# Wang-Xiaoyang/resource_packing_self_play

Hardware: AMD Instinct MI355X
Metric: self-play episodes/sec (with MCTS node expansions/sec alongside) (higher is better)
Workload: dtype f64 PUCT / f32 Q + CNN, u32 bit-board

## Files before the change

resource_packing_self_play_amd/csrc/rp_engine.hip:

```cpp
#include <hip/hip_runtime.h>
#include <math.h>
#include <stdarg.h>
#include <stdint.h>
#include <stdio.h>
#include <stdlib.h>
#include <string.h>

#include <algorithm>
#include <string>
#include <utility>
#include <vector>

#include "../../include/rp_engine.h"

#pragma clang fp contract(off)

typedef unsigned long long u64;
typedef unsigned int u32;
typedef unsigned short u16;
typedef unsigned char u8;

#define NONE32 0xFFFFFFFFu
#define NSA_MASK 0x3FFFFFFFu
#define WAVES_PER_BLOCK 4
// ... 2615 lines not shown
                if constexpr (e == 0 || T::L.s[e > 0 ? e - 1 : 0] != s) {
                    constexpr int s2 = s + 2;
                    const int off = s2 < 18 ? fbase + s2 * 2048 : fnext + (s2 - 18) * 2048;
                    wq[s2 % 3][0] = rs_load_b(frs, voff, off); wq[s2 % 3][1] = rs_load_b(frs, voff, off + 1024);
                }
                if constexpr (e + 2 < NE) bq[(e + 2) % 3] = b_read(std::integral_constant<int, (e + 2 < NE ? e + 2 : 0)>{});
                const f32x4 w0 = wq[s % 3][0], w1 = wq[s % 3][1], b = bq[e % 3];
                __builtin_amdgcn_sched_barrier(0);
#pragma unroll
                for (int j = 0; j < 4; ++j) {
                    acc[k][0] = __builtin_amdgcn_mfma_f32_16x16x4f32(w0[j], b[j], acc[k][0], 0, 0, 0);
                    acc[k][1] = __builtin_amdgcn_mfma_f32_16x16x4f32(w1[j], b[j], acc[k][1], 0, 0, 0);
                }
                __builtin_amdgcn_sched_barrier(0);
            });
            pm_sync<S>();
            const f32x4 ba = *(const f32x4 *)(sbias + 32 * kc + 4 * g), bb = *(const f32x4 *)(sbias + 32 * kc + 16 + 4 * g);
            if (kc < 3) {
                if (kc == 1)
                    pm_for<NP>([&](auto K) {
                        constexpr int k = decltype(K)::value, p = T::L.pos[k];
                        xs[k][0] = (acc[k][0] + ba) + xs[k][0]; xs[k][1] = (acc[k][1] + bb) + xs[k][1];
                        *(f32x4 *)(wb0 + p * 512) = rs_relu(xs[k][0]); *(f32x4 *)(wb1 + p * 512) = rs_relu(xs[k][1]);
                        __builtin_amdgcn_sched_barrier(0);
                    });
                else
                    pm_for<NP>([&](auto K) {
                        constexpr int k = decltype(K)::value, p = T::L.pos[k];
                        *(f32x4 *)(wb0 + p * 512) = rs_relu(acc[k][0] + ba); *(f32x4 *)(wb1 + p * 512) = rs_relu(acc[k][1] + bb);
                        __builtin_amdgcn_sched_barrier(0);
                    });
                pm_sync<S>();
            } else {
                const __amdgpu_buffer_rsrc_t ors = __builtin_amdgcn_make_buffer_rsrc((void *)(out + (size_t)leaf0 * PIX * 32), 0, nbytes, RS_BUF_FLAGS);
                pm_for<NP>([&](auto K) {
                    constexpr int k = decltype(K)::value, p = T::L.pos[k];
                    acc[k][0] = (acc[k][0] + ba) + xs[k][0]; acc[k][1] = (acc[k][1] + bb) + xs[k][1];
                    __builtin_amdgcn_raw_buffer_store_b128(__builtin_bit_cast(u32x4, acc[k][0]), ors, xoff, p * 128, RS_STREAM_AUX);
                    __builtin_amdgcn_raw_buffer_store_b128(__builtin_bit_cast(u32x4, acc[k][1]), ors, xoff, p * 128 + 64, RS_STREAM_AUX);
                    __builtin_amdgcn_sched_barrier(0);
                });
                if (out_relu != nullptr) {
                    const __amdgpu_buffer_rsrc_t rrs = __builtin_amdgcn_make_buffer_rsrc((void *)(out_relu + (size_t)leaf0 * PIX * 32), 0, nbytes, RS_BUF_FLAGS);
                    pm_for<NP>([&](auto K) {
                        constexpr int k = decltype(K)::value, p = T::L.pos[k];
                        __builtin_amdgcn_raw_buffer_store_b128(__builtin_bit_cast(u32x4, rs_relu(acc[k][0])), rrs, xoff, p * 128, RS_STREAM_AUX);
                        __builtin_amdgcn_raw_buffer_store_b128(__builtin_bit_cast(u32x4, rs_relu(acc[k][1])), rrs, xoff, p * 128 + 64, RS_STREAM_AUX);
                        __builtin_amdgcn_sched_barrier(0);
                    });
                }
            }
        }
    }
}
template <int S>
__global__ void __launch_bounds__(256, 2) k_resstage32_pm(const float *__restrict__ x, const float *__restrict__ frag, const float *__restrict__ bias,
                                                          float *__restrict__ out, float *__restrict__ out_relu, long long B, const int *__restrict__ nrows_dev) {
    extern __shared__ __attribute__((aligned(16))) float rb_lds[];
    const int wv = wave_in_block();
    if (nrows_dev) { const long long n = *nrows_dev; if (n < B) B = n; }
    float *sbias = rb_lds;
    if constexpr (S == 3) {
        if ((long long)blockIdx.x * 64 >= B) return;
        for (int i = threadIdx.x; i < 128; i += blockDim.x) sbias[i] = bias[i];
        __syncthreads();
        const long long leaf0 = ((long long)blockIdx.x * 4 + wv) * 16;
        if (leaf0 >= B) return;
        pm_body<3, 0>(x, frag, out, out_relu, B, leaf0, (long long)gridDim.x * 64, sbias, rb_lds + 128 + (size_t)wv * PM_IMG_FLOATS(3));
    } else {
        if ((long long)blockIdx.x * 16 >= B) return;
        for (int i = threadIdx.x; i < 128; i += blockDim.x) sbias[i] = bias[i];
        __syncthreads();
        const long long leaf0 = (long long)blockIdx.x * 16, stride = (long long)gridDim.x * 16;
        float *img = rb_lds + 128;
        switch (wv) {
            case 0: pm_body<5, 0>(x, frag, out, out_relu, B, leaf0, stride, sbias, img); break;
            case 1: pm_body<5, 1>(x, frag, out, out_relu, B, leaf0, stride, sbias, img); break;
            case 2: pm_body<5, 2>(x, frag, out, out_relu, B, leaf0, stride, sbias, img); break;
            default: pm_body<5, 3>(x, frag, out, out_relu, B, leaf0, stride, sbias, img); break;
        }
    }
}

#define CP_PS 36
#ifdef CP_STAMP
__device__ unsigned long long g_cp_stamp[8];
#endif
template <int NT, int CIN, bool TAIL = false>
__global__ void __launch_bounds__(256, 2) k_convpool32(const float *__restrict__ x, const float *__restrict__ frag, const float *__restrict__ bias,
                                                       float *__restrict__ out, long long B, int S_h, int S_w, int IMGW, int wave_floats,
                                                       const int *__restrict__ nrows_dev) {
    constexpr int XQ = CIN / 16;
    constexpr int PS = CP_PS;
    extern __shared__ __attribute__((aligned(16))) float rb_lds[];
    const int lane = lane_id(), wv = wave_in_block();
    if (nrows_dev) { const long long n = *nrows_dev; if (n < B) B = n; }
    if (((long long)blockIdx.x * 4) * IMGW >= B) return;
    const int PW = r32_pw(S_w), PIX = S_h * S_w, IMGP = r32_imgp(S_h, S_w), MP = IMGW * PIX;
    const int Hp = (S_h + 1) >> 1, Wp = (S_w + 1) >> 1, PP = Hp * Wp;
    constexpr int NTT = NT + (TAIL ? 1 : 0);
    int *ptab = (int *)rb_lds;
    int *pool = ptab + 16 * NTT;
    float *img = rb_lds + 16 * NTT + ((IMGW * PP + 3) & ~3) + (size_t)wv * wave_floats;
    for (int i = threadIdx.x; i < 16 * NTT; i += blockDim.x) {
        int im = i / PIX, pq = i - im * PIX, r = pq / S_w, c = pq - r * S_w;
        ptab[i] = i < MP ? im * IMGP + (r + 1) * PW + c + 1 : 0;
    }
    for (int i = threadIdx.x; i < IMGW * PP; i += blockDim.x) {
        int im = i / PP, pp = i - im * PP, pr = pp / Wp, px = pp - pr * Wp;
        pool[i] = (im * IMGP + (2 * pr + 1) * PW + 2 * px + 1) | ((pr > 0) << 16) | ((2 * pr + 1 < S_h) << 17) | ((px > 0) << 18) | ((2 * px + 1 < S_w) << 19);
    }
    {
        float4 *z4 = (float4 *)img;
        for (int i = lane; i < wave_floats / 4; i += 64) z4[i] = make_float4(0.f, 0.f, 0.f, 0.f);
    }
    __syncthreads();
    const long long stride_leaves = (long long)gridDim.x * 4 * IMGW;
    long long leaf0 = ((long long)blockIdx.x * 4 + wv) * IMGW;
    if (leaf0 >= B) return;
    const int n = lane & 15, g = lane >> 4;
    int abase[NT], pin[NT];
#pragma unroll
    for (int t = 0; t < NT; ++t) {
        const int m = t * 16 + n, pc = m < MP ? ptab[m] : IMGW * IMGP;
        abase[t] = (ptab[m < MP ? m : 0] - (PW + 1)) * PS + CIN / 4 * g;
        pin[t] = pc * PS + 4 * g;
    }
    const __amdgpu_buffer_rsrc_t frs = __builtin_amdgcn_make_buffer_rsrc((void *)frag, 0, 9 * CIN * 32 * 4, RS_BUF_FLAGS);
    const f32x4 ba = *(const f32x4 *)(bias + 4 * g), bb = *(const f32x4 *)(bias + 16 + 4 * g);
    const int rowoff = n * (CIN * 4) + g * 16;
    auto task_bytes = [&](long long l0) { return (int)(B - l0 < IMGW ? B - l0 : IMGW) * PIX * CIN * 4; };
    f32x4 xv[NT][XQ], wq[3][2];
    int t_abase = 0, t_voff0 = 0, t_voff1 = 0;
    f32x4 t_acc = (f32x4){0.f, 0.f, 0.f, 0.f}, t_w0[2], t_w1[2];
    const int cg = lane >> 3, kk = (lane >> 2) & 1, mt = 16 * NT + (lane & 3);
    int pout_t = 0, pin_t = 0;
    f32x4 xvt = (f32x4){0.f, 0.f, 0.f, 0.f};
    const int xq_t = (lane >> 2) & (CIN / 4 - 1);
    const int rowoff_t = (lane & 3) * (CIN * 4) + xq_t * 16;
    if (TAIL) {
        const int pc = mt < MP ? ptab[mt] : IMGW * IMGP;
        t_abase = (ptab[mt < MP ? mt : 0] - (PW + 1)) * PS + (CIN / 2) * kk;
        const int lw = 4 * (cg & 3) + (lane & 3) + 32 * kk;
        t_voff0 = (cg >> 2) * 1024 + lw * 16; t_voff1 = (cg >> 2) * 1024 + (lw + 16) * 16;
        pout_t = pc * PS + 4 * cg;
        pin_t = pc * PS + 4 * xq_t;
    }
    auto load_x = [&](long long l0) {
        const __amdgpu_buffer_rsrc_t rs = __builtin_amdgcn_make_buffer_rsrc((void *)(x + (size_t)l0 * PIX * CIN), 0, task_bytes(l0), RS_BUF_FLAGS);
#pragma unroll
        for (int t = 0; t < NT; ++t)
#pragma unroll
            for (int q = 0; q < XQ; ++q) xv[t][q] = rs_load_x(rs, rowoff, t * 16 * CIN * 4 + 64 * q);
        if (TAIL) xvt = rs_load_x(rs, rowoff_t, NT * 16 * CIN * 4);
    };
    const int cq = lane & 7;
    load_x(leaf0);
    wq[0][0] = rs_load_b(frs, lane * 16, 0); wq[0][1] = rs_load_b(frs, lane * 16, 1024);
    wq[1][0] = rs_load_b(frs, lane * 16, 2048); wq[1][1] = rs_load_b(frs, lane * 16, 3072);
    if (TAIL) {
        t_w0[0] = rs_load_b(frs, t_voff0, 0); t_w1[0] = rs_load_b(frs, t_voff1, 0);
        t_w0[1] = rs_load_b(frs, t_voff0, 2048); t_w1[1] = rs_load_b(frs, t_voff1, 2048);
    }
#ifdef CP_STAMP
    unsigned long long st_acc[8] = {0, 0, 0, 0, 0, 0, 0, 0}, st_last = __builtin_amdgcn_s_memtime();
#define CP_T(k) { unsigned long long now_ = __builtin_amdgcn_s_memtime(); st_acc[k] += now_ - st_last; st_last = now_; }
// ... 325 lines not shown
    u64 *meta_id;
    double *meta_bl;
    u8 *meta_has;
    int64_t meta_cap;
    int n_cu = 256;
    size_t lds_per_cu = 160 * 1024;
    int compact_rows = 0;
    const int *nn_rows_dev = nullptr;
    u16 *tr_action = nullptr, *fin_tr_action = nullptr;
    u64 *tr_rows = nullptr, *fin_tr_rows = nullptr, *fin_board = nullptr;
};

static std::string g_create_error;

static int fail(rp_ctx *ctx, int code, const char *fmt, ...) {
    char buf[512];
    va_list ap;
    va_start(ap, fmt);
    vsnprintf(buf, sizeof buf, fmt, ap);
    va_end(ap);
    if (ctx) ctx->err = buf; else g_create_error = buf;
    return code;
}
#define HIPCHK(ctx, call)                                                                              \
    do {                                                                                               \
        hipError_t e_ = (call);                                                                        \
        if (e_ != hipSuccess) return fail(ctx, RP_ERR_DEVICE, "%s failed: %s", #call, hipGetErrorString(e_)); \
    } while (0)

template <typename T> static int dev_alloc(rp_ctx *ctx, T **out, size_t n, bool zero = true) {
    void *ptr = nullptr;
    size_t bytes = std::max<size_t>(n, 1) * sizeof(T);
    HIPCHK(ctx, hipMalloc(&ptr, bytes));
    ctx->allocs.push_back(ptr);
    ctx->bytes += (int64_t)bytes;
    if (zero) HIPCHK(ctx, hipMemsetAsync(ptr, 0, bytes, ctx->stream));
    *out = (T *)ptr;
    return RP_OK;
}
#define ALLOC(ctx, ptr, n)                       \
    do {                                         \
        int rc_ = dev_alloc(ctx, &(ptr), (n));   \
        if (rc_ != RP_OK) return rc_;            \
    } while (0)

#define STAGE_BYTES(d) ((size_t)WAVES_PER_BLOCK * (size_t)(d).A * sizeof(u16))

#define STAGE_WAVES 2048
static int pick_leaves_per_wave(long long B, int PIX, int imgw_max) {
    const long long waves = STAGE_WAVES, typical = std::max<long long>(1, (long long)(0.92 * (double)B));
    long long best = -1;
    int pick = std::max(1, imgw_max);
    for (int k = std::max(1, imgw_max); k >= 1; --k) {
        const long long ntk = (k * PIX + 15) / 16;
        auto rounds = [&](long long rows) { const long long tasks = (rows + k - 1) / k; return (tasks + waves - 1) / waves; };
        const long long cost = (rounds(B) + 3 * rounds(typical)) * ntk;
        if (best < 0 || cost < best) { best = cost; pick = k; }
    }
    return pick;
}

static long long pm_rounds_cost(long long B, int k, long long units) {
    const long long typical = std::max<long long>(1, (long long)(0.92 * (double)B));
    auto rounds = [&](long long rows) { const long long tasks = (rows + k - 1) / k; return (tasks + units - 1) / units; };
    return rounds(B) + 3 * rounds(typical);
}
static size_t r32_wave_lds(int H, int W, int k) { return ((size_t)16 * ((k * H * W + 15) / 16) + 128 + 4 * ((size_t)k * r32_imgp(H, W) + 1) * r32_ps(32)) * sizeof(float); }
static void r32_wave_plan(long long B, int H, int W, int *imgw, int *nt) {
    const int PIX = H * W;
    int imgw_max = 80 / PIX;
    while (imgw_max > 1 && r32_wave_lds(H, W, imgw_max) > 78 * 1024) --imgw_max;
    *imgw = pick_leaves_per_wave(B, PIX, imgw_max);
    *nt = (*imgw * PIX + 15) / 16;
}
static bool stage32_pm_cheaper(long long B, int H, int W) {
    if (H != W || (H != 3 && H != 5) || B <= 0) return false;
    int imgw, nt;
    r32_wave_plan(B, H, W, &imgw, &nt);
    const long long cost_old = pm_rounds_cost(B, imgw, STAGE_WAVES) * nt * 9;
    const long long cost_pm = H == 3 ? pm_rounds_cost(B, 16, STAGE_WAVES) * 49 : pm_rounds_cost(B, 16, STAGE_WAVES / 4) * 43;
    return cost_pm < cost_old;
}

static long long wg_group_cost(long long B, int k, int tile_slots, int n_cu) {
    const long long typical = std::max<long long>(1, (long long)(0.92 * (double)B));
    auto rounds = [&](long long rows) { const long long tasks = (rows + k - 1) / k; return (tasks + n_cu - 1) / n_cu; };
    return (rounds(B) + 3 * rounds(typical)) * tile_slots;
}

enum { FAM_NONE, FAM_RS16, FAM_RS16_WG, FAM_RS32, FAM_RS32_WG, FAM_RS32_PM, FAM_CP, FAM_CP_WG };
enum { PLAN_OK, PLAN_BAD_SHAPE, PLAN_NO_LDS };
struct StagePlan { int family, nt, waves, cin, tail, imgw, wave_floats; size_t lds; unsigned grid, block; };
struct StageDevice { int n_cu; size_t lds_per_cu; };
struct StageKnobs { int wgs, tail, pm; };

static unsigned stage_grid(long long work, const StageDevice &dev, size_t lds, int wgs) {
    const int per_cu = (int)std::max<size_t>(1, std::min<size_t>((size_t)wgs, dev.lds_per_cu / lds));
    return (unsigned)std::min<long long>(work, (long long)dev.n_cu * per_cu);
}
static int plan_waves(StagePlan *p, long long B, int PIX, int imgw, size_t lds, const StageDevice &dev, int wgs, bool tail_ok) {
    p->imgw = imgw; p->nt = (imgw * PIX + 15) / 16; p->waves = 4; p->lds = lds; p->block = 256;
    if (lds > dev.lds_per_cu) return PLAN_NO_LDS;
    p->grid = stage_grid(((B + imgw - 1) / imgw + 3) / 4, dev, lds, wgs);
    const int tail_px = (imgw * PIX) & 15;
    if (tail_ok && p->nt == 7 && tail_px >= 1 && tail_px <= 4) { p->nt = 6; p->tail = 1; }
    return PLAN_OK;
}
template <class LdsOf> static int plan_wg_group(StagePlan *p, long long B, int PIX, int max_px, const StageDevice &dev, LdsOf lds_of) {
    long long best = -1;
    for (int k = 1; k * PIX <= max_px && lds_of(k) <= dev.lds_per_cu; ++k) {
        const int tk = (k * PIX + 15) / 16, wk = tk > 16 ? 8 : 4, ntk = (tk + wk - 1) / wk;
        const long long cost = wg_group_cost(B, k, wk * ntk, dev.n_cu);
        if (best < 0 || cost < best) { best = cost; p->imgw = k; p->nt = ntk; p->waves = wk; }
    }
    if (best < 0) return PLAN_NO_LDS;
    p->lds = lds_of(p->imgw); p->block = 64 * p->waves;
    p->grid = stage_grid((B + p->imgw - 1) / p->imgw, dev, p->lds, 2);
    return PLAN_OK;
}

static int plan_resstage16(StagePlan *p, long long B, int H, int W, const StageDevice &dev, const StageKnobs &kn) {
    *p = StagePlan{};
    if (B < 0 || H < 1 || W < 1 || H * W > 640) return PLAN_BAD_SHAPE;
    if (B == 0) return PLAN_OK;
    const int PIX = H * W;
    p->cin = 16;
    if (PIX > 128) {
        const int tiles = (PIX + 15) / 16;
        p->family = FAM_RS16_WG; p->imgw = 1; p->waves = tiles > 20 ? 8 : 4; p->nt = (tiles + p->waves - 1) / p->waves;
        p->lds = ((size_t)(H + 2) * (W + 2) * RS_STRIDE + RS_STRIDE) * sizeof(float); p->block = 64 * p->waves;
        if (p->lds > dev.lds_per_cu) return PLAN_NO_LDS;
        p->grid = stage_grid(B, dev, p->lds, 2);
        return PLAN_OK;
    }
    p->family = FAM_RS16;
    const size_t img_bytes = (size_t)(H + 2) * (W + 2) * RS_STRIDE * sizeof(float);
    int imgw_max = std::max(1, (16 * 8) / PIX);
    while (imgw_max > 1 && 4 * (imgw_max * img_bytes + RS_STRIDE * sizeof(float)) + 1024 > 78 * 1024) --imgw_max;
    const int imgw = pick_leaves_per_wave(B, PIX, imgw_max);
    return plan_waves(p, B, PIX, imgw, (size_t)16 * ((imgw * PIX + 15) / 16) * sizeof(int) + 4 * (imgw * img_bytes + RS_STRIDE * sizeof(float)), dev, kn.wgs, kn.tail != 0);
}

static int plan_convpool32(StagePlan *p, long long B, int Cin, int H, int W, const StageDevice &dev, const StageKnobs &kn) {
    *p = StagePlan{};
    if (B < 0 || H < 1 || W < 1 || (Cin != 16 && Cin != 32) || H * W > (Cin == 16 ? 640 : 512)) return PLAN_BAD_SHAPE;
    if (B == 0) return PLAN_OK;
    const int PIX = H * W;
    const size_t img_px = (size_t)r32_imgp(H, W);
    p->cin = Cin;
    if (PIX > (Cin == 16 ? 112 : 80)) {
        p->family = FAM_CP_WG;
        const int rc = plan_wg_group(p, B, PIX, Cin == 16 ? 640 : 512, dev, [&](int k) {
            return ((std::max<size_t>((k * img_px + 1) * r32_ps(Cin), (size_t)16 * ((k * PIX + 15) / 16) * 36) + 3) & ~(size_t)3) * sizeof(float); });
        p->wave_floats = (int)(p->lds / sizeof(float));
        return rc;
    }
    p->family = FAM_CP;
    const int PPn = ((H + 1) / 2) * ((W + 1) / 2);
    auto wave_floats = [&](int k) { return (size_t)(k * img_px + 1) * CP_PS; };
    auto lds_bytes = [&](int k) { return ((size_t)16 * ((k * PIX + 15) / 16) + (((size_t)k * PPn + 3) & ~(size_t)3) + 4 * wave_floats(k)) * sizeof(float); };
    int imgw = (16 * (Cin == 16 ? 7 : 5)) / PIX;
    while (imgw > 1 && lds_bytes(imgw) > 78 * 1024) --imgw;
    imgw = pick_leaves_per_wave(B, PIX, imgw);
    p->wave_floats = (int)wave_floats(imgw);
    return plan_waves(p, B, PIX, imgw, lds_bytes(imgw), dev, kn.wgs, kn.tail != 0 && Cin == 16);
}

static int plan_resstage32(StagePlan *p, long long B, int H, int W, const StageDevice &dev, const StageKnobs &kn) {
    *p = StagePlan{};
    if (B < 0 || H < 1 || W < 1 || H * W > 512) return PLAN_BAD_SHAPE;
    if (B == 0) return PLAN_OK;
    const int PIX = H * W;
    p->cin = 32;
    if (PIX > 80) {
        const size_t img_px = (size_t)r32_imgp(H, W);
        p->family = FAM_RS32_WG;
        return plan_wg_group(p, B, PIX, 512, dev, [&](int k) { return (128 + (k * img_px + 1) * r32_ps(32)) * sizeof(float); });
    }
    if (H == W && (H == 3 || H == 5) && (kn.pm == 1 || (kn.pm != 0 && stage32_pm_cheaper(B, H, W)))) {
        const long long tasks = (B + 15) / 16;
        p->family = FAM_RS32_PM; p->nt = PIX; p->waves = 4; p->imgw = 16; p->block = 256;
        p->lds = (128 + (size_t)(H == 3 ? 4 : 1) * PM_IMG_FLOATS(H)) * sizeof(float);
        p->grid = stage_grid(H == 3 ? (tasks + 3) / 4 : tasks, dev, p->lds, kn.wgs);
        return PLAN_OK;
    }
    p->family = FAM_RS32;
    int imgw, nt;
    r32_wave_plan(B, H, W, &imgw, &nt);
    return plan_waves(p, B, PIX, imgw, r32_wave_lds(H, W, imgw), dev, kn.wgs, false);
}

static StageKnobs stage_knobs(int entry) {
    auto env_int = [](const char *name, int unset) { const char *v = getenv(name); return v ? atoi(v) : unset; };
    static const int wgs[3] = {env_int("RP_STAGE16_WGS", 2), env_int("RP_CONVPOOL_WGS", 2), env_int("RP_STAGE32_WGS", 2)};
    static const int tail[3] = {env_int("RP_STAGE16_TAIL", 1), env_int("RP_CONVPOOL_TAIL", 1), 0};
    return StageKnobs{wgs[entry], tail[entry], entry == 2 ? env_int("RP_STAGE32_PM", -1) : -1};
}

extern "C" int rp_debug_stage_plan(int32_t entry, int32_t Cin, int64_t B, int32_t H, int32_t W, int32_t n_cu, int64_t lds_per_cu, int32_t wgs, int32_t tail,
                                   int32_t pm_force, int64_t *out) {
    StagePlan p{};
    const StageDevice dev{n_cu, (size_t)lds_per_cu};
    const StageKnobs kn{wgs, tail, pm_force};
    const int rc = entry == 0 ? plan_resstage16(&p, B, H, W, dev, kn) : entry == 1 ? plan_convpool32(&p, B, Cin, H, W, dev, kn) : plan_resstage32(&p, B, H, W, dev, kn);
    if (rc != PLAN_OK) p = StagePlan{};
    const int64_t f[10] = {p.family, p.nt, p.waves, p.cin, p.tail, p.imgw, p.wave_floats, (int64_t)p.lds, p.grid, p.block};
    std::copy(f, f + 10, out);
    return rc;
}
extern "C" int rp_debug_stage32_pm_pick(int64_t B, int32_t H, int32_t W) {
    StagePlan p;
    return plan_resstage32(&p, B, H, W, StageDevice{256, 160 * 1024}, StageKnobs{2, 0, -1}) == PLAN_OK && p.family == FAM_RS32_PM;
}
extern "C" int rp_debug_stage32_pm_swz(int32_t n) { return pm_swz(n); }

static int grid_for(long long waves) { return (int)((waves + WAVES_PER_BLOCK - 1) / WAVES_PER_BLOCK); }

static int allow_lds(rp_ctx *ctx, const void *fn, size_t lds, const char *what) {
    if (lds > ctx->lds_per_cu) return fail(ctx, RP_ERR_ARG, "%s: needs %zu bytes of LDS per workgroup, the device has %zu per CU", what, lds, ctx->lds_per_cu);
    if (lds <= 64 * 1024) return RP_OK;
    const hipError_t e = hipFuncSetAttribute(fn, hipFuncAttributeMaxDynamicSharedMemorySize, (int)lds);
    if (e != hipSuccess) return fail(ctx, RP_ERR_DEVICE, "%s: hipFuncSetAttribute(MaxDynamicSharedMemorySize = %zu) failed: %s", what, lds, hipGetErrorString(e));
    return RP_OK;
}

static int check_device_error(rp_ctx *ctx) {
    int e = 0;
    HIPCHK(ctx, hipMemcpyAsync(&e, ctx->d.error, sizeof(int), hipMemcpyDeviceToHost, ctx->stream));
    HIPCHK(ctx, hipStreamSynchronize(ctx->stream));
    if (e == 0) return RP_OK;
    (void)hipMemsetAsync(ctx->d.error, 0, sizeof(int), ctx->stream);
    static const char *names[] = {"", "node arena overflow (raise node_cap)", "legal-move arena overflow (raise edge_cap)",
                                  "transposition table full", "action is not a legal move of the (expanded) root", "search path broken",
                                  "finished-episode ring overflow", "replay buffer full (raise max_examples / max_sparse)",
                                  "visited-edge arena overflow (raise vis_cap)", "replay example index or sparse entry outside the packed arrays"};
    int code = (e == ERR_BAD_ACTION) ? RP_ERR_ASSERT : (e == ERR_PATH ? RP_ERR_STATE : (e == ERR_BAD_EXAMPLE ? RP_ERR_ARG : RP_ERR_CAPACITY));
    return fail(ctx, code, "device error %d: %s", e, e < 10 ? names[e] : "?");
}

static int build_plan(int lo, int n, std::vector<int> &llo, std::vector<int> &ln, std::vector<int> &sd, std::vector<int> &ss) {
    if (n <= 128) {
        llo.push_back(lo); ln.push_back(n);
        return (int)llo.size() - 1;
    }
    int n2 = n / 2;
    n2 -= n2 % 8;
    int a = build_plan(lo, n2, llo, ln, sd, ss);
    int b = build_plan(lo + n2, n - n2, llo, ln, sd, ss);
    sd.push_back(a); ss.push_back(b);
    return a;
}

extern "C" int rp_version(void) { return RP_ABI_VERSION; }

extern "C" const char *rp_last_error(const rp_ctx *ctx) { return ctx ? ctx->err.c_str() : g_create_error.c_str(); }

extern "C" int64_t rp_device_bytes(const rp_ctx *ctx) { return ctx ? ctx->bytes : 0; }

extern "C" void rp_destroy(rp_ctx *ctx) {
    if (!ctx) return;
    (void)hipSetDevice(ctx->cfg.device);
    (void)hipStreamSynchronize(ctx->stream);
    for (void *p : ctx->allocs) (void)hipFree(p);
    delete ctx;
}

extern "C" int rp_create(const rp_config *cfg, rp_ctx **out) {
    if (!cfg || !out) return fail(nullptr, RP_ERR_ARG, "null argument");
    *out = nullptr;
    if (cfg->abi_version != RP_ABI_VERSION) return fail(nullptr, RP_ERR_ARG, "abi_version %d != %d", cfg->abi_version, RP_ABI_VERSION);
    if (cfg->W < 1 || cfg->W > 64 || cfg->H < 1 || cfg->H > 64 || cfg->N < 1 || cfg->N > 128)
        return fail(nullptr, RP_ERR_ARG, "limits: 1<=W<=64, 1<=H<=64, 1<=N<=128 (got %d %d %d)", cfg->W, cfg->H, cfg->N);
    if (cfg->games < 1 || cfg->sims < 0) return fail(nullptr, RP_ERR_ARG, "games >= 1 and sims >= 0 required");
    if (!(cfg->cpuct > 0.0)) return fail(nullptr, RP_ERR_ARG, "cpuct must be positive (got %g): the best unvisited move of a node is kept as the one with the largest prior, which is the PUCT winner among the unvisited moves only for cpuct > 0", cfg->cpuct);
    if ((int64_t)cfg->sims * (cfg->N + 1) >= (int64_t)NSA_MASK) return fail(nullptr, RP_ERR_ARG, "sims too large");
    int ndev = 0;
    if (hipGetDeviceCount(&ndev) != hipSuccess || ndev <= cfg->device)
        return fail(nullptr, RP_ERR_DEVICE, "no HIP device %d (found %d): the engine has no CPU fallback", cfg->device, ndev);
    rp_ctx *ctx = new rp_ctx();
    ctx->cfg = *cfg;
    ctx->bytes = 0;
    ctx->fin_popped = 0;
    ctx->pool_wh = nullptr; ctx->pool_area = nullptr; ctx->pool_max_h = nullptr; ctx->pool_cap = 0;
    ctx->meta_id = nullptr; ctx->meta_bl = nullptr; ctx->meta_has = nullptr; ctx->meta_cap = 0;
    ctx->stream = (hipStream_t)cfg->stream;
    hipError_t e = hipSetDevice(cfg->device);
    if (e != hipSuccess) { delete ctx; return fail(nullptr, RP_ERR_DEVICE, "hipSetDevice: %s", hipGetErrorString(e)); }
    {
        hipDeviceProp_t prop;
        if (hipGetDeviceProperties(&prop, cfg->device) == hipSuccess) {
            if (prop.multiProcessorCount > 0) ctx->n_cu = prop.multiProcessorCount;
            size_t lds = strstr(prop.gcnArchName, "gfx950") ? (size_t)160 * 1024 : (size_t)64 * 1024;
            if (prop.maxSharedMemoryPerMultiProcessor > lds) lds = prop.maxSharedMemoryPerMultiProcessor;
            ctx->lds_per_cu = lds;
        }
// ... 405 lines not shown
        if (t_lds) hipLaunchKernelGGL((k_leaf_stem<u32, true>), dim3(grid), dim3(64 * WAVES_PER_BLOCK), t_bytes, ctx->stream, d, out_dev, out_relu_dev, (long long)capacity_rows, (int)(channels_last != 0));
        else hipLaunchKernelGGL((k_leaf_stem<u32, false>), dim3(grid), dim3(64 * WAVES_PER_BLOCK), 0, ctx->stream, d, out_dev, out_relu_dev, (long long)capacity_rows, (int)(channels_last != 0));
    }
    HIPCHK(ctx, hipGetLastError());
    return RP_OK;
}

extern "C" int rp_nn_bias_relu(rp_ctx *ctx, float *x_dev, const float *bias_dev, int64_t B, int32_t C, int32_t HW) {
    if (!ctx || !x_dev || !bias_dev || B < 0 || C < 1 || HW < 1) return fail(ctx, RP_ERR_ARG, "rp_nn_bias_relu: bad argument");
    long long n = (long long)B * C * HW;
    if (n % 4) return fail(ctx, RP_ERR_ARG, "rp_nn_bias_relu: element count must be a multiple of 4");
    if (n == 0) return RP_OK;
    hipLaunchKernelGGL(k_nn_bias_relu, dim3((unsigned)((n / 4 + 255) / 256)), dim3(256), 0, ctx->stream, x_dev, bias_dev, n / 4, (int)C, (int)HW);
    HIPCHK(ctx, hipGetLastError());
    return RP_OK;
}

extern "C" int rp_nn_bias_residual(rp_ctx *ctx, const float *x_dev, const float *bias_dev, const float *res_dev, float *out_dev, float *out_relu_dev,
                                   int64_t B, int32_t C, int32_t HW) {
    if (!ctx || !x_dev || !bias_dev || !res_dev || !out_dev || B < 0 || C < 1 || HW < 1) return fail(ctx, RP_ERR_ARG, "rp_nn_bias_residual: bad argument");
    long long n = (long long)B * C * HW;
    if (n % 4) return fail(ctx, RP_ERR_ARG, "rp_nn_bias_residual: element count must be a multiple of 4");
    if (n == 0) return RP_OK;
    hipLaunchKernelGGL(k_nn_bias_residual, dim3((unsigned)((n / 4 + 255) / 256)), dim3(256), 0, ctx->stream, x_dev, bias_dev, res_dev, out_dev, out_relu_dev,
                       n / 4, (int)C, (int)HW);
    HIPCHK(ctx, hipGetLastError());
    return RP_OK;
}

extern "C" int rp_nn_bias_pool(rp_ctx *ctx, const float *x_dev, const float *bias_dev, float *out_dev, float *out_relu_dev, int64_t B, int32_t C, int32_t H,
                               int32_t W, int32_t channels_last) {
    if (!ctx || !x_dev || !bias_dev || !out_dev || B < 0 || C < 1 || H < 1 || W < 1) return fail(ctx, RP_ERR_ARG, "rp_nn_bias_pool: bad argument");
    int Hp = (H + 1) / 2, Wp = (W + 1) / 2;
    long long n = (long long)B * C * Hp * Wp;
    if (n == 0) return RP_OK;
    if (channels_last && C % 4 == 0 && n / 4 < 0xFFFFFF00LL)
        hipLaunchKernelGGL(k_nn_bias_pool_nhwc4, dim3((unsigned)((n / 4 + 255) / 256)), dim3(256), 0, ctx->stream, (const float4 *)x_dev, (const float4 *)bias_dev,
                           (float4 *)out_dev, (float4 *)out_relu_dev, (unsigned)(n / 4), (unsigned)(C / 4), (int)H, (int)W, Hp, Wp);
    else if (channels_last)
        hipLaunchKernelGGL(k_nn_bias_pool_nhwc, dim3((unsigned)((n + 255) / 256)), dim3(256), 0, ctx->stream, x_dev, bias_dev, out_dev, out_relu_dev, n, (int)C,
                           (int)H, (int)W, Hp, Wp);
    else
        hipLaunchKernelGGL(k_nn_bias_pool, dim3((unsigned)((n + 255) / 256)), dim3(256), 0, ctx->stream, x_dev, bias_dev, out_dev, out_relu_dev, n, (int)C, (int)H,
                           (int)W, Hp, Wp);
    HIPCHK(ctx, hipGetLastError());
    return RP_OK;
}

extern "C" int rp_nn_value_head(rp_ctx *ctx, const float *z_dev, const float *w_dev, const float *bias_dev, float *out_dev, int64_t B, int32_t K) {
    if (!ctx || !z_dev || !w_dev || !bias_dev || !out_dev || B < 0 || K < 4 || K % 4) return fail(ctx, RP_ERR_ARG, "rp_nn_value_head: bad argument (K a multiple of 4)");
    if (B == 0) return RP_OK;
    hipLaunchKernelGGL(k_nn_value_head, dim3((unsigned)((B + 3) / 4)), dim3(256), 0, ctx->stream, (const float4 *)z_dev, (const float4 *)w_dev, bias_dev, out_dev,
                       (long long)B, (int)(K / 4));
    HIPCHK(ctx, hipGetLastError());
    return RP_OK;
}

extern "C" int rp_nn_pack_conv16(rp_ctx *ctx, const float *w_dev, float *frag_dev) {
    if (!ctx || !w_dev || !frag_dev) return fail(ctx, RP_ERR_ARG, "rp_nn_pack_conv16: bad argument");
    hipLaunchKernelGGL(k_pack_conv16, dim3(9), dim3(256), 0, ctx->stream, w_dev, frag_dev);
    HIPCHK(ctx, hipGetLastError());
    return RP_OK;
}

extern "C" int rp_nn_resblock16(rp_ctx *ctx, const float *x_dev, const float *frag0_dev, const float *bias0_dev, const float *frag1_dev, const float *bias1_dev,
                                float *out_dev, float *out_relu_dev, int64_t B, int32_t H, int32_t W) {
    if (!ctx || !x_dev || !frag0_dev || !bias0_dev || !frag1_dev || !bias1_dev || !out_dev || B < 0 || H < 1 || W < 1 || H > 62 || W > 62)
        return fail(ctx, RP_ERR_ARG, "rp_nn_resblock16: bad argument");
    if (B == 0) return RP_OK;
    const size_t lds = ((size_t)4 * 2 * (H + 2) * (W + 2) * RB_STRIDE + (((size_t)H * W + 3) & ~(size_t)3)) * sizeof(float);
    { const int rc = allow_lds(ctx, (const void *)k_resblock16, lds, "rp_nn_resblock16"); if (rc != RP_OK) return rc; }
    const int per_cu = (int)std::max<size_t>(1, std::min<size_t>(4, ctx->lds_per_cu / lds));
    const int grid = (int)std::min<long long>((B + 3) / 4, (long long)ctx->n_cu * per_cu);
    hipLaunchKernelGGL(k_resblock16, dim3(grid), dim3(256), lds, ctx->stream, x_dev, frag0_dev, bias0_dev, frag1_dev, bias1_dev, out_dev, out_relu_dev, (long long)B,
                       (int)H, (int)W);
    HIPCHK(ctx, hipGetLastError());
    return RP_OK;
}

template <class Fn> struct StageEntry { int nt, waves, cin, tail; Fn fn; };
typedef void (*StageFn)(const float *, const float *, const float *, float *, float *, long long, int, int, int, const int *);
typedef void (*StageWg16Fn)(const float *, const float *, const float *, float *, float *, long long, int, int, const int *);
typedef void (*StagePmFn)(const float *, const float *, const float *, float *, float *, long long, const int *);
typedef void (*ConvPoolFn)(const float *, const float *, const float *, float *, long long, int, int, int, int, const int *);
template <int NT, bool TAIL = false> constexpr StageEntry<StageFn> rs16() { return {NT, 4, 16, TAIL, k_resstage16<NT, TAIL>}; }
template <int NT, int WV> constexpr StageEntry<StageWg16Fn> rs16_wg() { return {NT, WV, 16, 0, k_resstage16_wg<NT, WV>}; }
template <int NT> constexpr StageEntry<StageFn> rs32() { return {NT, 4, 32, 0, k_resstage32<NT>}; }
template <int NT, int WV> constexpr StageEntry<StageFn> rs32_wg() { return {NT, WV, 32, 0, k_resstage32_wg<NT, WV>}; }
template <int S> constexpr StageEntry<StagePmFn> rs32_pm() { return {S * S, 4, 32, 0, k_resstage32_pm<S>}; }
template <int NT, int CIN, bool TAIL = false> constexpr StageEntry<ConvPoolFn> cp() { return {NT, 4, CIN, TAIL, k_convpool32<NT, CIN, TAIL>}; }
template <int NT, int CIN, int WV> constexpr StageEntry<ConvPoolFn> cp_wg() { return {NT, WV, CIN, 0, k_convpool32_wg<NT, CIN, WV>}; }
static const StageEntry<StageWg16Fn> RS16_WG_TABLE[] = {rs16_wg<3, 4>(), rs16_wg<4, 4>(), rs16_wg<5, 4>(), rs16_wg<3, 8>(), rs16_wg<4, 8>(), rs16_wg<5, 8>()};
static const StageEntry<StageFn> RS16_TABLE[] = {rs16<6, true>(), rs16<1>(), rs16<2>(), rs16<3>(), rs16<4>(), rs16<5>(), rs16<6>(), rs16<7>(), rs16<8>()};
static const StageEntry<ConvPoolFn> CP_WG_TABLE[] = {cp_wg<2, 16, 4>(), cp_wg<3, 16, 4>(), cp_wg<4, 16, 4>(), cp_wg<3, 16, 8>(), cp_wg<4, 16, 8>(), cp_wg<5, 16, 8>(),
                                                     cp_wg<2, 32, 4>(), cp_wg<3, 32, 4>(), cp_wg<4, 32, 4>(), cp_wg<3, 32, 8>(), cp_wg<4, 32, 8>()};
static const StageEntry<ConvPoolFn> CP_TABLE[] = {cp<6, 16, true>(), cp<1, 16>(), cp<2, 16>(), cp<3, 16>(), cp<4, 16>(), cp<5, 16>(), cp<6, 16>(), cp<7, 16>(),
                                                  cp<1, 32>(), cp<2, 32>(), cp<3, 32>(), cp<4, 32>(), cp<5, 32>()};
static const StageEntry<StageFn> RS32_WG_TABLE[] = {rs32_wg<2, 4>(), rs32_wg<3, 4>(), rs32_wg<4, 4>(), rs32_wg<3, 8>(), rs32_wg<4, 8>()};
static const StageEntry<StagePmFn> RS32_PM_TABLE[] = {rs32_pm<3>(), rs32_pm<5>()};
static const StageEntry<StageFn> RS32_TABLE[] = {rs32<1>(), rs32<2>(), rs32<3>(), rs32<4>(), rs32<5>()};

template <class... P, size_t N, class... A>
static int launch_stage(rp_ctx *ctx, const char *what, const StagePlan &p, const StageEntry<void (*)(P...)> (&table)[N], A... args) {
    for (const auto &e : table) {
        if (e.nt != p.nt || e.waves != p.waves || e.cin != p.cin || e.tail != p.tail) continue;
        { const int rc = allow_lds(ctx, (const void *)e.fn, p.lds, what); if (rc != RP_OK) return rc; }
        hipLaunchKernelGGL(e.fn, dim3(p.grid), dim3(p.block), p.lds, ctx->stream, args...);
        HIPCHK(ctx, hipGetLastError());
        return RP_OK;
    }
    return fail(ctx, RP_ERR_ARG, "%s: unsupported image size", what);
}
static int plan_error(rp_ctx *ctx, int rc, const char *what, const char *limits, int H, int W, const StagePlan &p) {
    if (rc == PLAN_BAD_SHAPE) return fail(ctx, RP_ERR_ARG, "%s: bad argument (%s)", what, limits);
    if (p.lds == 0) return fail(ctx, RP_ERR_ARG, "%s: a %dx%d image does not fit LDS", what, H, W);
    return fail(ctx, RP_ERR_ARG, "%s: a %dx%d image needs %zu bytes of LDS%s, the device has %zu per CU", what, H, W, p.lds, p.family == FAM_RS16_WG ? "" : " per workgroup",
                ctx->lds_per_cu);
}

extern "C" int rp_nn_resstage16(rp_ctx *ctx, const float *x_dev, const float *frag4_dev, const float *bias4_dev, float *out_dev, float *out_relu_dev, int64_t B,
                                int32_t H, int32_t W) {
    const char *what = "rp_nn_resstage16";
    StagePlan p{};
    const int rc = !ctx || !x_dev || !frag4_dev || !bias4_dev || !out_dev ? PLAN_BAD_SHAPE : plan_resstage16(&p, B, H, W, StageDevice{ctx->n_cu, ctx->lds_per_cu}, stage_knobs(0));
    if (rc != PLAN_OK) return plan_error(ctx, rc, what, "images of at most 640 pixels", H, W, p);
    if (B == 0) return RP_OK;
    if (p.family == FAM_RS16_WG) return launch_stage(ctx, what, p, RS16_WG_TABLE, x_dev, frag4_dev, bias4_dev, out_dev, out_relu_dev, B, H, W, ctx->nn_rows_dev);
    return launch_stage(ctx, what, p, RS16_TABLE, x_dev, frag4_dev, bias4_dev, out_dev, out_relu_dev, B, H, W, p.imgw, ctx->nn_rows_dev);
}

extern "C" int rp_nn_pack_conv32(rp_ctx *ctx, const float *w_dev, float *frag_dev, int32_t Cin) {
    if (!ctx || !w_dev || !frag_dev || (Cin != 16 && Cin != 32)) return fail(ctx, RP_ERR_ARG, "rp_nn_pack_conv32: bad argument (Cin 16 or 32)");
    const int n = 9 * Cin * 32;
    hipLaunchKernelGGL(k_pack_conv32, dim3((n + 255) / 256), dim3(256), 0, ctx->stream, w_dev, frag_dev, (int)Cin);
    HIPCHK(ctx, hipGetLastError());
    return RP_OK;
}

extern "C" int rp_nn_convpool32(rp_ctx *ctx, const float *x_dev, const float *frag_dev, const float *bias_dev, float *out_dev, int64_t B, int32_t Cin, int32_t H,
                                int32_t W) {
    const char *what = "rp_nn_convpool32";
    StagePlan p{};
    const int rc = !ctx || !x_dev || !frag_dev || !bias_dev || !out_dev ? PLAN_BAD_SHAPE : plan_convpool32(&p, B, Cin, H, W, StageDevice{ctx->n_cu, ctx->lds_per_cu}, stage_knobs(1));
    if (rc != PLAN_OK) return plan_error(ctx, rc, what, "Cin 16: <= 640 pixels, Cin 32: <= 512 pixels", H, W, p);
    if (B == 0) return RP_OK;
    if (p.family == FAM_CP_WG) return launch_stage(ctx, what, p, CP_WG_TABLE, x_dev, frag_dev, bias_dev, out_dev, B, H, W, p.imgw, p.wave_floats, ctx->nn_rows_dev);
    return launch_stage(ctx, what, p, CP_TABLE, x_dev, frag_dev, bias_dev, out_dev, B, H, W, p.imgw, p.wave_floats, ctx->nn_rows_dev);
}

extern "C" int rp_nn_resstage32(rp_ctx *ctx, const float *x_dev, const float *frag4_dev, const float *bias4_dev, float *out_dev, float *out_relu_dev, int64_t B,
                                int32_t H, int32_t W) {
    const char *what = "rp_nn_resstage32";
    StagePlan p{};
    const int rc = !ctx || !x_dev || !frag4_dev || !bias4_dev || !out_dev ? PLAN_BAD_SHAPE : plan_resstage32(&p, B, H, W, StageDevice{ctx->n_cu, ctx->lds_per_cu}, stage_knobs(2));
    if (rc != PLAN_OK) return plan_error(ctx, rc, what, "images of at most 512 pixels", H, W, p);
    if (B == 0) return RP_OK;
    if (p.family == FAM_RS32_PM) return launch_stage(ctx, what, p, RS32_PM_TABLE, x_dev, frag4_dev, bias4_dev, out_dev, out_relu_dev, B, ctx->nn_rows_dev);
    if (p.family == FAM_RS32_WG) return launch_stage(ctx, what, p, RS32_WG_TABLE, x_dev, frag4_dev, bias4_dev, out_dev, out_relu_dev, B, H, W, p.imgw, ctx->nn_rows_dev);
    return launch_stage(ctx, what, p, RS32_TABLE, x_dev, frag4_dev, bias4_dev, out_dev, out_relu_dev, B, H, W, p.imgw, ctx->nn_rows_dev);
}

extern "C" int rp_leaf_states(rp_ctx *ctx, int32_t max_rows, uint64_t *rows_out, uint8_t *remaining_out, int32_t *slot_out, int32_t *n_out) {
    if (!ctx || max_rows < 0 || !rows_out || !remaining_out || !slot_out || !n_out) return fail(ctx, RP_ERR_ARG, "rp_leaf_states: bad argument");
    const DP &d = ctx->d;
    if (d.rows_identity) return fail(ctx, RP_ERR_STATE, "rp_leaf_states: call rp_search_step with n_leaves_out first (compact rows)");
    int n = 0;
    HIPCHK(ctx, hipMemcpyAsync(&n, d.eval_count, sizeof(int), hipMemcpyDeviceToHost, ctx->stream));
    HIPCHK(ctx, hipStreamSynchronize(ctx->stream));
    n = std::min(n, (int)max_rows);
    *n_out = n;
    if (n == 0) return RP_OK;
    Scratch s(ctx);
    u64 *drows = s.up((const u64 *)nullptr, (size_t)n * d.H); NEED(drows);
    u8 *drem = s.up((const u8 *)nullptr, (size_t)n * d.N); NEED(drem);
    int *dslot = s.up((const int *)nullptr, (size_t)n); NEED(dslot);
    DISPATCH(ctx, k_leaf_states, grid_for(n), d, drows, drem, dslot, n);
    HIPCHK(ctx, hipMemcpyAsync(rows_out, drows, (size_t)n * d.H * 8, hipMemcpyDeviceToHost, ctx->stream));
    HIPCHK(ctx, hipMemcpyAsync(remaining_out, drem, (size_t)n * d.N, hipMemcpyDeviceToHost, ctx->stream));
    HIPCHK(ctx, hipMemcpyAsync(slot_out, dslot, (size_t)n * sizeof(int), hipMemcpyDeviceToHost, ctx->stream));
    HIPCHK(ctx, hipStreamSynchronize(ctx->stream));
    return RP_OK;
}

static int launch_commit(rp_ctx *ctx, const float *pi_dev, const float *v_dev, bool logits) {
    const DP &d = ctx->d;
    const dim3 grid(grid_for(d.G)), block(64 * WAVES_PER_BLOCK);
    const size_t lds = (size_t)WAVES_PER_BLOCK * ((size_t)d.n_leaves * sizeof(double) + (size_t)std::min(d.A, TERM_CHUNK) * sizeof(float) +
                                                 (logits ? (size_t)d.A * sizeof(float) : 0) + (size_t)(((d.A + 31) >> 5) + 1) * sizeof(u32));
    if (logits) {
        if (ctx->row64) hipLaunchKernelGGL((k_commit<u64, true>), grid, block, lds, ctx->stream, d, pi_dev, v_dev);
        else hipLaunchKernelGGL((k_commit<u32, true>), grid, block, lds, ctx->stream, d, pi_dev, v_dev);
    } else {
        if (ctx->row64) hipLaunchKernelGGL((k_commit<u64, false>), grid, block, lds, ctx->stream, d, pi_dev, v_dev);
        else hipLaunchKernelGGL((k_commit<u32, false>), grid, block, lds, ctx->stream, d, pi_dev, v_dev);
    }
    hipError_t le_ = hipGetLastError();
    if (le_ != hipSuccess) return fail(ctx, RP_ERR_DEVICE, "launch of k_commit failed: %s", hipGetErrorString(le_));
    return RP_OK;
}

extern "C" int rp_commit_eval(rp_ctx *ctx, const float *pi_dev, const float *v_dev) {
    if (!ctx || !pi_dev || !v_dev) return fail(ctx, RP_ERR_ARG, "rp_commit_eval: bad argument");
    return launch_commit(ctx, pi_dev, v_dev, false);
}

extern "C" int rp_commit_eval_logits(rp_ctx *ctx, const float *logits_dev, const float *v_dev) {
    if (!ctx || !logits_dev || !v_dev) return fail(ctx, RP_ERR_ARG, "rp_commit_eval_logits: bad argument");
    if ((size_t)WAVES_PER_BLOCK * ctx->d.A * sizeof(float) > 24 * 1024)
        return fail(ctx, RP_ERR_ARG, "rp_commit_eval_logits: %d actions do not fit the kernel's LDS row buffers (at most 1536): take the softmax first and call rp_commit_eval", ctx->d.A);
    return launch_commit(ctx, logits_dev, v_dev, true);
}

extern "C" int rp_commit_eval_host(rp_ctx *ctx, const float *pi_host, const float *v_host, int32_t n_rows) {
    if (!ctx || !pi_host || !v_host || n_rows < 0) return fail(ctx, RP_ERR_ARG, "rp_commit_eval_host: bad argument");
    const DP &d = ctx->d;
    if (d.rows_identity) return fail(ctx, RP_ERR_STATE, "rp_commit_eval_host: call rp_search_step with n_leaves_out first (compact rows)");
    int n = 0;
    HIPCHK(ctx, hipMemcpyAsync(&n, d.eval_count, sizeof(int), hipMemcpyDeviceToHost, ctx->stream));
    HIPCHK(ctx, hipStreamSynchronize(ctx->stream));
    if (n_rows < n) return fail(ctx, RP_ERR_ARG, "rp_commit_eval_host: %d rows given, %d leaves waiting", n_rows, n);
    if (n == 0) return RP_OK;
    Scratch s(ctx);
    float *dpi = s.up(pi_host, (size_t)n * d.A); NEED(dpi);
    float *dv = s.up(v_host, (size_t)n); NEED(dv);
    { const int rc = launch_commit(ctx, dpi, dv, false); if (rc != RP_OK) return rc; }
    HIPCHK(ctx, hipStreamSynchronize(ctx->stream));
    return check_device_error(ctx);
}
// ... 426 lines not shown
```

Baseline: 1537.

## Add pixel-major MFMA conv+maxpool kernel for 5x5 Cin=32 stage

```diff
diff --git a/resource_packing_self_play_amd/csrc/rp_engine.hip b/resource_packing_self_play_amd/csrc/rp_engine.hip
--- a/resource_packing_self_play_amd/csrc/rp_engine.hip
+++ b/resource_packing_self_play_amd/csrc/rp_engine.hip
@@ -2721,6 +2721,133 @@
     }
 }
 
+__host__ __device__ constexpr int cp_pm_out(int role, int i) {
+    constexpr int t[4][3] = {{4, 0, -1}, {1, 3, -1}, {5, 7, -1}, {2, 6, 8}};
+    return i < 3 ? t[role][i] : -1;
+}
+__host__ __device__ constexpr int cp_pm_win(int pp, int i) {
+    const int r = 2 * (pp / 3) - 1 + i / 3, c = 2 * (pp % 3) - 1 + i % 3;
+    return (r >= 0 && r < 5 && c >= 0 && c < 5) ? r * 5 + c : -1;
+}
+constexpr int cp_pm_reads(int role) {
+    int n = 0;
+    for (int o = 0; o < 3 && cp_pm_out(role, o) >= 0; ++o)
+        for (int i = 0; i < 9; ++i) n += cp_pm_win(cp_pm_out(role, o), i) >= 0;
+    return n;
+}
+constexpr bool cp_pm_covers() {
+    int outs[9] = {}, seen[25] = {};
+    for (int role = 0; role < 4; ++role)
+        for (int o = 0; o < 3 && cp_pm_out(role, o) >= 0; ++o) {
+            ++outs[cp_pm_out(role, o)];
+            for (int i = 0; i < 9; ++i)
+                if (cp_pm_win(cp_pm_out(role, o), i) >= 0) ++seen[cp_pm_win(cp_pm_out(role, o), i)];
+        }
+    for (int i = 0; i < 9; ++i) if (outs[i] != 1) return false;
+    for (int i = 0; i < 25; ++i) if (seen[i] < 1) return false;
+    return true;
+}
+static_assert(cp_pm_reads(0) + cp_pm_reads(1) + cp_pm_reads(2) + cp_pm_reads(3) == 49 && cp_pm_covers(), "5x5 -> 3x3 pooling: nine windows, 49 reads");
+#define CP_PM_LDS_BYTES (PM_IMG_FLOATS(5) * sizeof(float))
+template <int ROLE>
+__device__ __forceinline__ void cp_pm_body(const float *__restrict__ x, const float *__restrict__ frag, const float *__restrict__ bias, float *__restrict__ out,
+                                           long long B, long long leaf0, long long stride_leaves, float *img) {
+    using T = PmTab<5, ROLE>;
+    constexpr int NP = T::L.np, NE = T::L.n, PIX = 25, PP = 9, CONV_BYTES = 9 * 32 * 32 * 4;
+    const int lane = lane_id(), n = lane & 15, g = lane >> 4, sw = pm_swz(n);
+    const float *rb0 = img + n * 32 + 4 * ((2 * g) ^ sw), *rb1 = img + n * 32 + 4 * ((2 * g + 1) ^ sw);
+    float *wb0 = img + n * 32 + 4 * (g ^ sw), *wb1 = img + n * 32 + 4 * ((4 + g) ^ sw);
+    const int voff = lane * 16, xoff = n * (PIX * 128) + g * 16, ooff = n * (PP * 128) + g * 16;
+    const __amdgpu_buffer_rsrc_t frs = __builtin_amdgcn_make_buffer_rsrc((void *)frag, 0, CONV_BYTES, RS_BUF_FLAGS);
+    const f32x4 ba = *(const f32x4 *)(bias + 4 * g), bb = *(const f32x4 *)(bias + 16 + 4 * g);
+    f32x4 xs[NP][2], acc[NP][2], wq[3][2], bq[3];
+    auto load_x = [&](long long l0) {
+        const int nb = (int)(B - l0 < 16 ? B - l0 : 16) * PIX * 128;
+        const __amdgpu_buffer_rsrc_t xrs = __builtin_amdgcn_make_buffer_rsrc((void *)(x + (size_t)l0 * PIX * 32), 0, nb, RS_BUF_FLAGS);
+        pm_for<NP>([&](auto K) {
+            constexpr int k = decltype(K)::value, p = T::L.pos[k];
+            xs[k][0] = rs_load_x(xrs, xoff, p * 128); xs[k][1] = rs_load_x(xrs, xoff, p * 128 + 64);
+        });
+    };
+    auto b_read = [&](auto E) {
+        constexpr int e = decltype(E)::value, off = T::L.q[e] * 512;
+        return *(const f32x4 *)(((T::L.s[e] & 1) ? rb1 : rb0) + off);
+    };
+    load_x(leaf0);
+    wq[0][0] = rs_load_b(frs, voff, 0); wq[0][1] = rs_load_b(frs, voff, 1024);
+    wq[1][0] = rs_load_b(frs, voff, 2048); wq[1][1] = rs_load_b(frs, voff, 3072);
+    for (; leaf0 < B; leaf0 += stride_leaves) {
+        pm_for<NP>([&](auto K) {
+            constexpr int k = decltype(K)::value, p = T::L.pos[k];
+            *(f32x4 *)(wb0 + p * 512) = xs[k][0]; *(f32x4 *)(wb1 + p * 512) = xs[k][1];
+            __builtin_amdgcn_sched_barrier(0);
+        });
+        if (leaf0 + stride_leaves < B) load_x(leaf0 + stride_leaves);
+        lds_barrier();
+        pm_for<NP>([&](auto K) {
+            constexpr int k = decltype(K)::value;
+            acc[k][0] = (f32x4){0.f, 0.f, 0.f, 0.f}; acc[k][1] = (f32x4){0.f, 0.f, 0.f, 0.f};
+        });
+        bq[0] = b_read(std::integral_constant<int, 0>{}); bq[1] = b_read(std::integral_constant<int, 1>{});
+        pm_for<NE>([&](auto E) {
+            constexpr int e = decltype(E)::value, s = T::L.s[e], k = T::L.k[e];
+            if constexpr (e == 0 || T::L.s[e > 0 ? e - 1 : 0] != s) {
+                constexpr int s2 = s + 2, off = (s2 < 18 ? s2 : s2 - 18) * 2048;
+                wq[s2 % 3][0] = rs_load_b(frs, voff, off); wq[s2 % 3][1] = rs_load_b(frs, voff, off + 1024);
+            }
+            if constexpr (e + 2 < NE) bq[(e + 2) % 3] = b_read(std::integral_constant<int, (e + 2 < NE ? e + 2 : 0)>{});
+            const f32x4 w0 = wq[s % 3][0], w1 = wq[s % 3][1], b = bq[e % 3];
+            __builtin_amdgcn_sched_barrier(0);
+#pragma unroll
+            for (int j = 0; j < 4; ++j) {
+                acc[k][0] = __builtin_amdgcn_mfma_f32_16x16x4f32(w0[j], b[j], acc[k][0], 0, 0, 0);
+                acc[k][1] = __builtin_amdgcn_mfma_f32_16x16x4f32(w1[j], b[j], acc[k][1], 0, 0, 0);
+            }
+            __builtin_amdgcn_sched_barrier(0);
+        });
+        lds_barrier();
+        pm_for<NP>([&](auto K) {
+            constexpr int k = decltype(K)::value, p = T::L.pos[k];
+            *(f32x4 *)(wb0 + p * 512) = acc[k][0] + ba; *(f32x4 *)(wb1 + p * 512) = acc[k][1] + bb;
+            __builtin_amdgcn_sched_barrier(0);
+        });
+        lds_barrier();
+        const int obytes = (int)(B - leaf0 < 16 ? B - leaf0 : 16) * PP * 128;
+        const __amdgpu_buffer_rsrc_t ors = __builtin_amdgcn_make_buffer_rsrc((void *)(out + (size_t)leaf0 * PP * 32), 0, obytes, RS_BUF_FLAGS);
+        pm_for<3>([&](auto O) {
+            constexpr int pp = cp_pm_out(ROLE, decltype(O)::value);
+            if constexpr (pp >= 0) {
+                f32x4 m0 = *(const f32x4 *)(wb0 + cp_pm_win(pp, 4) * 512), m1 = *(const f32x4 *)(wb1 + cp_pm_win(pp, 4) * 512);
+                pm_for<9>([&](auto I) {
+                    constexpr int q = cp_pm_win(pp, decltype(I)::value);
+                    if constexpr (q >= 0 && decltype(I)::value != 4) {
+                        const f32x4 v0 = *(const f32x4 *)(wb0 + q * 512), v1 = *(const f32x4 *)(wb1 + q * 512);
+#pragma unroll
+                        for (int j = 0; j < 4; ++j) { m0[j] = fmaxf(m0[j], v0[j]); m1[j] = fmaxf(m1[j], v1[j]); }
+                    }
+                });
+                __builtin_amdgcn_raw_buffer_store_b128(__builtin_bit_cast(u32x4, m0), ors, ooff, pp * 128, RS_STREAM_AUX);
+                __builtin_amdgcn_raw_buffer_store_b128(__builtin_bit_cast(u32x4, m1), ors, ooff, pp * 128 + 64, RS_STREAM_AUX);
+            }
+        });
+        lds_barrier();
+    }
+}
+__global__ void __launch_bounds__(256, 2) k_convpool32_pm(const float *__restrict__ x, const float *__restrict__ frag, const float *__restrict__ bias,
+                                                          float *__restrict__ out, long long B, const int *__restrict__ nrows_dev) {
+    extern __shared__ __attribute__((aligned(16))) float rb_lds[];
+    const int wv = wave_in_block();
+    if (nrows_dev) { const long long n = *nrows_dev; if (n < B) B = n; }
+    if ((long long)blockIdx.x * 16 >= B) return;
+    const long long leaf0 = (long long)blockIdx.x * 16, stride = (long long)gridDim.x * 16;
+    switch (wv) {
+        case 0: cp_pm_body<0>(x, frag, bias, out, B, leaf0, stride, rb_lds); break;
+        case 1: cp_pm_body<1>(x, frag, bias, out, B, leaf0, stride, rb_lds); break;
+        case 2: cp_pm_body<2>(x, frag, bias, out, B, leaf0, stride, rb_lds); break;
+        default: cp_pm_body<3>(x, frag, bias, out, B, leaf0, stride, rb_lds); break;
+    }
+}
+
 #define CP_PS 36
 #ifdef CP_STAMP
 __device__ unsigned long long g_cp_stamp[8];
@@ -3212,17 +3339,23 @@
     return cost_pm < cost_old;
 }
 
+static bool convpool32_pm_cheaper(long long B, int imgw) {
+    if (B <= 0) return false;
+    const int nt = (imgw * 25 + 15) / 16;
+    return pm_rounds_cost(B, 16, STAGE_WAVES / 4) * 43 < pm_rounds_cost(B, imgw, STAGE_WAVES) * nt * 9;
+}
+
 static long long wg_group_cost(long long B, int k, int tile_slots, int n_cu) {
     const long long typical = std::max<long long>(1, (long long)(0.92 * (double)B));
     auto rounds = [&](long long rows) { const long long tasks = (rows + k - 1) / k; return (tasks + n_cu - 1) / n_cu; };
     return (rounds(B) + 3 * rounds(typical)) * tile_slots;
 }
 
-enum { FAM_NONE, FAM_RS16, FAM_RS16_WG, FAM_RS32, FAM_RS32_WG, FAM_RS32_PM, FAM_CP, FAM_CP_WG };
+enum { FAM_NONE, FAM_RS16, FAM_RS16_WG, FAM_RS32, FAM_RS32_WG, FAM_RS32_PM, FAM_CP, FAM_CP_WG, FAM_CP_PM };
 enum { PLAN_OK, PLAN_BAD_SHAPE, PLAN_NO_LDS };
 struct StagePlan { int family, nt, waves, cin, tail, imgw, wave_floats; size_t lds; unsigned grid, block; };
 struct StageDevice { int n_cu; size_t lds_per_cu; };
-struct StageKnobs { int wgs, tail, pm; };
+struct StageKnobs { int wgs, tail, pm, cp_pm; };
 
 static unsigned stage_grid(long long work, const StageDevice &dev, size_t lds, int wgs) {
     const int per_cu = (int)std::max<size_t>(1, std::min<size_t>((size_t)wgs, dev.lds_per_cu / lds));
@@ -3292,6 +3425,12 @@
     int imgw = (16 * (Cin == 16 ? 7 : 5)) / PIX;
     while (imgw > 1 && lds_bytes(imgw) > 78 * 1024) --imgw;
     imgw = pick_leaves_per_wave(B, PIX, imgw);
+    if (Cin == 32 && H == 5 && W == 5 && CP_PM_LDS_BYTES <= dev.lds_per_cu && (kn.cp_pm == 1 || (kn.cp_pm != 0 && convpool32_pm_cheaper(B, imgw)))) {
+        p->family = FAM_CP_PM; p->nt = PIX; p->waves = 4; p->imgw = 16; p->block = 256;
+        p->lds = CP_PM_LDS_BYTES;
+        p->grid = stage_grid((B + 15) / 16, dev, p->lds, kn.wgs);
+        return PLAN_OK;
+    }
     p->wave_floats = (int)wave_floats(imgw);
     return plan_waves(p, B, PIX, imgw, lds_bytes(imgw), dev, kn.wgs, kn.tail != 0 && Cin == 16);
 }
@@ -3324,23 +3463,32 @@
     auto env_int = [](const char *name, int unset) { const char *v = getenv(name); return v ? atoi(v) : unset; };
     static const int wgs[3] = {env_int("RP_STAGE16_WGS", 2), env_int("RP_CONVPOOL_WGS", 2), env_int("RP_STAGE32_WGS", 2)};
     static const int tail[3] = {env_int("RP_STAGE16_TAIL", 1), env_int("RP_CONVPOOL_TAIL", 1), 0};
-    return StageKnobs{wgs[entry], tail[entry], entry == 2 ? env_int("RP_STAGE32_PM", -1) : -1};
+    return StageKnobs{wgs[entry], tail[entry], entry == 2 ? env_int("RP_STAGE32_PM", -1) : -1, entry == 1 ? env_int("RP_CONVPOOL_PM", -1) : 0};
 }
 
 extern "C" int rp_debug_stage_plan(int32_t entry, int32_t Cin, int64_t B, int32_t H, int32_t W, int32_t n_cu, int64_t lds_per_cu, int32_t wgs, int32_t tail,
                                    int32_t pm_force, int64_t *out) {
     StagePlan p{};
     const StageDevice dev{n_cu, (size_t)lds_per_cu};
-    const StageKnobs kn{wgs, tail, pm_force};
+    const StageKnobs kn{wgs, tail, pm_force, 0};
     const int rc = entry == 0 ? plan_resstage16(&p, B, H, W, dev, kn) : entry == 1 ? plan_convpool32(&p, B, Cin, H, W, dev, kn) : plan_resstage32(&p, B, H, W, dev, kn);
     if (rc != PLAN_OK) p = StagePlan{};
     const int64_t f[10] = {p.family, p.nt, p.waves, p.cin, p.tail, p.imgw, p.wave_floats, (int64_t)p.lds, p.grid, p.block};
     std::copy(f, f + 10, out);
     return rc;
 }
+extern "C" int rp_debug_convpool_plan(int32_t Cin, int64_t B, int32_t H, int32_t W, int32_t n_cu, int64_t lds_per_cu, int32_t wgs, int32_t tail, int32_t cp_pm,
+                                      int64_t *out) {
+    StagePlan p{};
+    const int rc = plan_convpool32(&p, B, Cin, H, W, StageDevice{n_cu, (size_t)lds_per_cu}, StageKnobs{wgs, tail, -1, cp_pm});
+    if (rc != PLAN_OK) p = StagePlan{};
+    const int64_t f[10] = {p.family, p.nt, p.waves, p.cin, p.tail, p.imgw, p.wave_floats, (int64_t)p.lds, p.grid, p.block};
+    std::copy(f, f + 10, out);
+    return rc;
+}
 extern "C" int rp_debug_stage32_pm_pick(int64_t B, int32_t H, int32_t W) {
     StagePlan p;
-    return plan_resstage32(&p, B, H, W, StageDevice{256, 160 * 1024}, StageKnobs{2, 0, -1}) == PLAN_OK && p.family == FAM_RS32_PM;
+    return plan_resstage32(&p, B, H, W, StageDevice{256, 160 * 1024}, StageKnobs{2, 0, -1, 0}) == PLAN_OK && p.family == FAM_RS32_PM;
 }
 extern "C" int rp_debug_stage32_pm_swz(int32_t n) { return pm_swz(n); }
 
@@ -3912,6 +4060,7 @@
 typedef void (*StageFn)(const float *, const float *, const float *, float *, float *, long long, int, int, int, const int *);
 typedef void (*StageWg16Fn)(const float *, const float *, const float *, float *, float *, long long, int, int, const int *);
 typedef void (*StagePmFn)(const float *, const float *, const float *, float *, float *, long long, const int *);
+typedef void (*ConvPoolPmFn)(const float *, const float *, const float *, float *, long long, const int *);
 typedef void (*ConvPoolFn)(const float *, const float *, const float *, float *, long long, int, int, int, int, const int *);
 template <int NT, bool TAIL = false> constexpr StageEntry<StageFn> rs16() { return {NT, 4, 16, TAIL, k_resstage16<NT, TAIL>}; }
 template <int NT, int WV> constexpr StageEntry<StageWg16Fn> rs16_wg() { return {NT, WV, 16, 0, k_resstage16_wg<NT, WV>}; }
@@ -3926,6 +4075,7 @@
                                                      cp_wg<2, 32, 4>(), cp_wg<3, 32, 4>(), cp_wg<4, 32, 4>(), cp_wg<3, 32, 8>(), cp_wg<4, 32, 8>()};
 static const StageEntry<ConvPoolFn> CP_TABLE[] = {cp<6, 16, true>(), cp<1, 16>(), cp<2, 16>(), cp<3, 16>(), cp<4, 16>(), cp<5, 16>(), cp<6, 16>(), cp<7, 16>(),
                                                   cp<1, 32>(), cp<2, 32>(), cp<3, 32>(), cp<4, 32>(), cp<5, 32>()};
+static const StageEntry<ConvPoolPmFn> CP_PM_TABLE[] = {{25, 4, 32, 0, k_convpool32_pm}};
 static const StageEntry<StageFn> RS32_WG_TABLE[] = {rs32_wg<2, 4>(), rs32_wg<3, 4>(), rs32_wg<4, 4>(), rs32_wg<3, 8>(), rs32_wg<4, 8>()};
 static const StageEntry<StagePmFn> RS32_PM_TABLE[] = {rs32_pm<3>(), rs32_pm<5>()};
 static const StageEntry<StageFn> RS32_TABLE[] = {rs32<1>(), rs32<2>(), rs32<3>(), rs32<4>(), rs32<5>()};
@@ -3974,6 +4124,7 @@
     const int rc = !ctx || !x_dev || !frag_dev || !bias_dev || !out_dev ? PLAN_BAD_SHAPE : plan_convpool32(&p, B, Cin, H, W, StageDevice{ctx->n_cu, ctx->lds_per_cu}, stage_knobs(1));
     if (rc != PLAN_OK) return plan_error(ctx, rc, what, "Cin 16: <= 640 pixels, Cin 32: <= 512 pixels", H, W, p);
     if (B == 0) return RP_OK;
+    if (p.family == FAM_CP_PM) return launch_stage(ctx, what, p, CP_PM_TABLE, x_dev, frag_dev, bias_dev, out_dev, B, ctx->nn_rows_dev);
     if (p.family == FAM_CP_WG) return launch_stage(ctx, what, p, CP_WG_TABLE, x_dev, frag_dev, bias_dev, out_dev, B, H, W, p.imgw, p.wave_floats, ctx->nn_rows_dev);
     return launch_stage(ctx, what, p, CP_TABLE, x_dev, frag_dev, bias_dev, out_dev, B, H, W, p.imgw, p.wave_floats, ctx->nn_rows_dev);
 }
```

After: 1565 (median of 6 runs). 1.8% higher.
